# schmidtjonathan/Climate2Weather

Hardware: AMD Instinct MI355X
Metric: UNet denoise steps/sec (train fwd+bwd+allreduce+AdamW+EMA windows/s) (higher is better)
Workload: dtype bf16; 1 GPU; configs/sda_unet.yml default net, 5 vars x window 13 = 65 ch, 128x128, bf16 training step, 128 windows/GPU/step; global_batch=128, parallelism=dp1, params=72132929

## Files before the change

climate2weather_amd/_lib.py:

```python
from __future__ import annotations

import ctypes
import os
from ctypes import POINTER, Structure, c_char_p, c_float, c_int, c_int32, c_longlong, c_ulonglong, c_void_p

HERE = os.path.dirname(os.path.abspath(__file__))
LIB_PATH = os.environ.get("C2W_LIB") or os.path.join(HERE, "libc2w_hip.so")

DTYPE_F32, DTYPE_BF16, DTYPE_F16 = 0, 1, 2
CONV_1X1, CONV_S1, CONV_S2, CONV_UP, CONV_TS2 = 0, 1, 2, 3, 4
ACT_NONE, ACT_SILU, ACT_SILU_PAIR, ACT_RELU, ACT_RELU_PAIR = 0, 1, 2, 3, 4
MUL_PLAIN, MUL_DSILU = 0, 1
CONV_POOL2, CONV_WPACKED, CONV_NO_Y = 1, 2, 4
KERNEL_GATHER, KERNEL_PATCH_8X16, KERNEL_PATCH_16X16, KERNEL_PATCH_PAIR, KERNEL_PATCH_TS2, KERNEL_PATCH_S2 = 0, 1, 2, 3, 4, 5


class C2wError(RuntimeError):
    pass


class ConvArgs(Structure):
    _fields_ = [
        ("x", c_void_p), ("w", c_void_p), ("bias", c_void_p), ("res", c_void_p), ("mul", c_void_p), ("y", c_void_p), ("y2", c_void_p),
        ("B", c_int32), ("Hin", c_int32), ("Win", c_int32), ("Cin", c_int32),
        ("Hout", c_int32), ("Wout", c_int32), ("Cout", c_int32), ("ldy", c_int32),
        ("wrows", c_int32), ("mode", c_int32), ("act", c_int32), ("mulmode", c_int32),
        ("ln_x", c_void_p), ("ln_m", c_void_p), ("ln_dm", c_void_p), ("ln_ldm", c_int32), ("ln_unbiased", c_int32),
        ("ln_eps", c_float), ("flags", c_int32), ("lnf_y", c_void_p), ("lnf_m", c_void_p), ("kvalid", c_int32),
        ("lnf_rstd", c_void_p), ("ln_rstd", c_void_p),
        ("lnf_mean", c_void_p), ("res_rstd", c_void_p), ("res_mean", c_void_p), ("res_m", c_void_p),
        ("loss_sum", c_void_p), ("loss_scaler", c_void_p), ("loss_eps", c_void_p), ("loss_gscale", c_float), ("loss_C", c_int32),
        ("loss_lde", c_int32), ("splitk_ws", c_void_p), ("splitk_ws_bytes", c_ulonglong), ("splitk", c_int32),
    ]


class WgradItem(Structure):
    _fields_ = [("x", c_void_p), ("dy", c_void_p), ("dw", c_void_p), ("dbias", c_void_p)]


_PROTOS = {
    "c2w_conv_forward": [POINTER(ConvArgs), c_int, c_int, c_void_p],
    "c2w_conv_lnbwd_supported": [POINTER(ConvArgs), c_int],
    "c2w_conv_lnfwd_supported": [POINTER(ConvArgs), c_int],
    "c2w_conv_loss_supported": [POINTER(ConvArgs), c_int],
    "c2w_conv_splitk_plan": [POINTER(ConvArgs), c_int, POINTER(c_ulonglong)],
    "c2w_conv_lnfwd_chain_supported": [POINTER(ConvArgs), c_int],
    "c2w_conv_patch_supported": [POINTER(ConvArgs), c_int],
# ... 23 lines not shown
    "c2w_windows_to_nhwc_noise": [c_void_p, c_void_p, c_ulonglong, c_void_p, c_void_p, c_int, c_int, c_int, c_int, c_int, c_void_p],
    "c2w_mse_loss_grad_noise": [c_void_p, c_ulonglong, c_void_p, c_void_p, c_int, c_int, c_int, c_int, c_float, c_void_p, c_int, c_void_p],
    "c2w_sq_err": [c_void_p, c_void_p, c_void_p, c_void_p, c_int, c_int, c_int, c_int, c_int, c_void_p],
    "c2w_sq_err_noise": [c_void_p, c_ulonglong, c_void_p, c_void_p, c_int, c_int, c_int, c_int, c_int, c_void_p],
    "c2w_timestep_embedding": [c_void_p, c_void_p, c_int, c_int, c_float, c_void_p],
    "c2w_mu_sigma": [c_void_p, c_void_p, c_int, c_float, c_void_p],
    "c2w_publish_scalar": [c_void_p, c_void_p, c_int, c_void_p],
    "c2w_gemv_f32": [c_void_p, c_void_p, c_void_p, c_void_p, c_int, c_int, c_int, c_int, c_void_p],
    "c2w_conv_center_supported": [c_int, c_int, c_int, c_int, c_int],
    "c2w_conv_center": [c_void_p, c_void_p, c_void_p, c_void_p, c_int, c_int, c_int, c_int, c_int, c_int, c_int, c_longlong, c_int, c_void_p],
    "c2w_cast_f32": [c_void_p, c_void_p, c_longlong, c_int, c_void_p],
    "c2w_weight_transpose": [c_void_p, c_void_p, c_int, c_int, c_int, c_int, c_int, c_int, c_int, c_void_p],
    "c2w_weight_transpose_batched": [c_void_p, c_void_p, c_void_p, c_int, c_int, c_void_p],
    "c2w_pack_conv_weights_batched": [c_void_p, c_void_p, c_void_p, c_int, c_int, c_void_p],
    "c2w_conv_wpacked_supported": [POINTER(ConvArgs), c_int],
    "c2w_adamw_ema": [c_void_p, c_void_p, c_void_p, c_void_p, c_void_p, c_void_p, c_longlong, c_float, c_float, c_float, c_float,
                      c_float, c_int, c_float, c_float, c_void_p],
    "c2w_adamw_ema_scaled": [c_void_p, c_void_p, c_void_p, c_void_p, c_void_p, c_void_p, c_int, c_longlong, c_float, c_float, c_float,
                             c_float, c_float, c_int, c_float, c_float, c_void_p, c_void_p],
    "c2w_grad_scaler_init": [c_void_p, c_float, c_void_p],
    "c2w_grad_scaler_check": [c_void_p, c_longlong, c_void_p, c_void_p],
    "c2w_grad_scaler_update": [c_void_p, c_float, c_float, c_int, c_void_p],
    "c2w_ema_update": [c_void_p, c_void_p, c_longlong, c_float, c_void_p],
    "c2w_attention_forward": [c_void_p, c_void_p, c_void_p, c_int, c_int, c_int, c_int, c_void_p],
    "c2w_attention_backward": [c_void_p, c_void_p, c_void_p, c_void_p, c_void_p, c_void_p, c_int, c_int, c_int, c_int, c_void_p],
    "c2w_window_gather": [c_void_p, c_void_p, c_int, c_int, c_int, c_int, c_int, c_int, c_int, c_void_p],
    "c2w_window_scatter": [c_void_p, c_void_p, c_int, c_int, c_int, c_int, c_int, c_int, c_int, c_int, c_void_p],
    "c2w_sampler_predict": [c_void_p, c_void_p, c_void_p, c_longlong, c_float, c_float, c_void_p],
    "c2w_sumsq": [c_void_p, c_void_p, c_longlong, c_void_p],
    "c2w_sampler_correct": [c_void_p, c_void_p, c_void_p, c_void_p, c_void_p, c_longlong, c_float, c_float, c_void_p],
# ... 56 lines not shown
```

climate2weather_amd/csrc/conv_igemm.hip:

```cpp
#include <cstdlib>

#include "conv_epilogue.h"
#include "knobs.h"

namespace {

constexpr int BN = 128;
constexpr int WBYTES = BN * 128;
constexpr int NSLOT = 3;
template <int NW> struct GCfg {
    static constexpr int BM = 64 * NW;
    static constexpr int NTHREADS = 128 * NW;
    static constexpr int PBYTES = BM * 128;
    static constexpr int ROWS_PER_ROUND = NTHREADS / 8;
    static constexpr int WROUNDS = BN / ROWS_PER_ROUND;
    static constexpr int ROUND_BYTES = NTHREADS * 16;
};

template <typename T> struct Mma;
template <> struct Mma<bf16_t> {
    __device__ static __forceinline__ void run(const u32x4_t& a, const u32x4_t& b, f32x4_t& c) { c = mfma16<bf16_t>(a, b, c); }
};
template <> struct Mma<f16_t> {
    __device__ static __forceinline__ void run(const u32x4_t& a, const u32x4_t& b, f32x4_t& c) { c = mfma16<f16_t>(a, b, c); }
// ... 354 lines not shown
    return c2w_knobs().ln_chain && a->mode == C2W_CONV_S1 && c2w_conv_patch3_wanted(*a, dtype) ? 1 : 0;
}

extern "C" int c2w_conv_loss_supported(const C2wConvArgs* a, int dtype) {
    if (a == nullptr || (dtype != C2W_DTYPE_BF16 && dtype != C2W_DTYPE_F16)) return 0;
    if (a->mode != C2W_CONV_S1 || a->wrows > 80 || a->Cout > 128 || a->ldy != 128 || a->res != nullptr || a->mul != nullptr || a->y2 != nullptr ||
        a->act != C2W_ACT_NONE || a->ln_x != nullptr || a->lnf_y != nullptr || (a->flags & C2W_CONV_POOL2) != 0)
        return 0;
    if (a->loss_sum != nullptr && (a->loss_eps == nullptr || a->loss_C <= 0 || a->loss_C > a->wrows || (a->loss_lde & 7) != 0 || a->loss_lde < a->loss_C ||
                                   a->loss_lde > 128))
        return 0;
    const C2wKnobs& k = c2w_knobs();
    return !k.force_gather && k.loss_fusion && k.wgrad_narrow && c2w_conv_patch_eligible(*a) && c2w_conv_patch3_wanted(*a, dtype) ? 1 : 0;
}

extern "C" int c2w_conv_wpacked_supported(const C2wConvArgs* a, int dtype) {
    if (a == nullptr || (dtype != C2W_DTYPE_BF16 && dtype != C2W_DTYPE_F16)) return 0;
    return !c2w_knobs().force_gather && c2w_knobs().wpacked && c2w_conv_patch_eligible(*a) && c2w_conv_patch3_wanted(*a, dtype) ? 1 : 0;
}

extern "C" int c2w_conv_dispatch(const C2wConvArgs* a, int dtype) {
    if (a == nullptr) return C2W_ERR_BAD_ARG;
    const bool gather = c2w_knobs().force_gather;
    if (!gather && c2w_conv_patch_eligible(*a)) return c2w_conv_patch3_wanted(*a, dtype) ? C2W_KERNEL_PATCH_16X16 : C2W_KERNEL_PATCH_8X16;
    if (!gather && c2w_conv_pair_eligible(*a)) return C2W_KERNEL_PATCH_PAIR;
    if (!gather && c2w_conv_ts2_patch_eligible(*a)) return C2W_KERNEL_PATCH_TS2;
    if (!gather && c2w_conv_s2_patch_eligible(*a, dtype)) return C2W_KERNEL_PATCH_S2;
    return C2W_KERNEL_GATHER;
}

// ... 12 lines not shown
    if (a->lnf_y != nullptr && (naive != 0 || !c2w_conv_lnfwd_supported(a, dtype))) return C2W_ERR_BAD_SHAPE;
    if ((a->ln_rstd != nullptr && a->ln_x == nullptr) || (a->lnf_rstd != nullptr && a->lnf_y == nullptr)) return C2W_ERR_BAD_ARG;
    if (a->lnf_mean != nullptr || a->res_rstd != nullptr || a->res_mean != nullptr || a->res_m != nullptr || (a->flags & C2W_CONV_NO_Y) != 0) {
        if (a->lnf_y == nullptr || (a->res_rstd == nullptr) != (a->res_mean == nullptr) || (a->res_m != nullptr && a->res_rstd == nullptr) ||
            (a->res_rstd != nullptr && a->res == nullptr))
            return C2W_ERR_BAD_ARG;
        if (naive != 0 || !c2w_conv_lnfwd_chain_supported(a, dtype)) return C2W_ERR_BAD_SHAPE;
    }
    if ((a->flags & C2W_CONV_POOL2) != 0 && (naive != 0 || !c2w_conv_pool2_supported(a, dtype))) return C2W_ERR_BAD_SHAPE;
    if (a->loss_sum != nullptr && (naive != 0 || !c2w_conv_loss_supported(a, dtype))) return C2W_ERR_BAD_SHAPE;
    if (a->splitk > 1) {
        unsigned long long need = 0;
        if (naive != 0 || a->splitk_ws == nullptr || c2w_conv_splitk_plan_impl(*a, dtype, &need) != a->splitk || a->splitk_ws_bytes < need) return C2W_ERR_BAD_SHAPE;
    }
    if ((a->flags & C2W_CONV_WPACKED) != 0 && (naive != 0 || !c2w_conv_wpacked_supported(a, dtype))) return C2W_ERR_BAD_SHAPE;
    const bool patch = naive == 0 && !c2w_knobs().force_gather;
    if (patch && c2w_conv_patch_eligible(*a)) return c2w_conv_patch_s1(*a, dtype, st);
    if (patch && c2w_conv_pair_eligible(*a)) return c2w_conv_patch_pair(*a, dtype, st);
    if (patch && c2w_conv_ts2_patch_eligible(*a)) return c2w_conv_patch_ts2(*a, dtype, st);
    if (patch && c2w_conv_s2_patch_eligible(*a, dtype)) return c2w_conv_patch_s2(*a, dtype, st);
    if (naive == 2) naive = 0;
    if (dtype == C2W_DTYPE_F32) return launch_dtype<float>(*a, naive, st);
    if (dtype == C2W_DTYPE_BF16) return launch_dtype<bf16_t>(*a, naive, st);
    if (dtype == C2W_DTYPE_F16) return launch_dtype<f16_t>(*a, naive, st);
    return C2W_ERR_BAD_ARG;
}
```

climate2weather_amd/csrc/conv_patch3.hip:

```cpp
#include <cstdlib>

#include "conv_epilogue.h"
#include "knobs.h"

namespace {

constexpr int T3_WAVES = 8;
constexpr int T3_PW = 20;
constexpr int T3_WBYTES = 128 * 64;
constexpr int T3_OS = 128 * 2 + 16;

template <int TR, int NW = 4> struct T3Cfg {
    static constexpr int NTHR = 64 * NW;
    static constexpr int NPIECE = ((TR + 2) * T3_PW + 7) / 8;
    static constexpr int PBYTES = NPIECE * 1024;
    static constexpr int ROUNDS = (NPIECE + NW - 1) / NW;
    static constexpr int WPIECES = 8 / NW;
    static constexpr int NB = TR / (2 * NW);
    static constexpr int NPASS = TR / 8;
    static constexpr int LDS_LOOP = PBYTES + 3 * T3_WBYTES;
    static constexpr int LDS_EPI = TR * 16 * T3_OS + 512;
    static constexpr int LDS_BIAS = LDS_LOOP > LDS_EPI ? LDS_LOOP : LDS_EPI;
    static constexpr int LDS = LDS_BIAS + 1024;
    static constexpr int WAVES_PER_SIMD = NW == 8 ? 4 : (TR == 8 ? 3 : 2);
    static_assert(NB >= 1 && 8 % NW == 0, "wave tiling");
// ... 2 lines not shown
template <int N> struct IC3 { static constexpr int value = N; };


__device__ __forceinline__ uint32_t t3_pswz(int col) { return (uint32_t)(col & 7); }
__device__ __forceinline__ uint32_t t3_wswz(int row) { return (uint32_t)((4 - ((row >> 2) & 3)) & 3); }

template <int WPIECES> __device__ __forceinline__ void t3_wait(bool more) {
    if (more) {
        if constexpr (WPIECES == 2) asm volatile("s_waitcnt vmcnt(2)" ::: "memory");
        else asm volatile("s_waitcnt vmcnt(1)" ::: "memory");
    } else {
        asm volatile("s_waitcnt vmcnt(0)" ::: "memory");
    }
}

template <int TR, typename T = bf16_t, int NW = 4, int EPI = 0, bool WPK = false>
__global__ __launch_bounds__(64 * NW, (T3Cfg<TR, NW>::WAVES_PER_SIMD)) void conv_patch_t3_kernel(const C2wConvArgs p) {
    static_assert(sizeof(T) == 2, "16-bit storage types only");
    typedef T3Cfg<TR, NW> CF;
    constexpr int T3_NTHR = CF::NTHR;
    constexpr int ESZ = 2;
    constexpr int NB = CF::NB;
    extern __shared__ __attribute__((aligned(16))) char smem[];

    const int tid = threadIdx.x;
    const int lane = tid & 63;
    const int wid = __builtin_amdgcn_readfirstlane(tid >> 6);
    const int li = lane & 15, lg = lane >> 4;
    constexpr bool NARROW = EPI == 5 || EPI == 7;
    const int wm = NARROW ? wid >> 2 : wid & 1, wn = NARROW ? wid & 3 : wid >> 1;
    const bool light = NARROW && wid >= 4;
// ... 45 lines not shown
        if (NARROW && wid >= 5) return;
        if constexpr (wpk) {
            const uint32_t so = (uint32_t)(((tap * (p.Cin >> 5) + chunk * 2 + half) * (nN * 128) + co0) * 64);
#pragma unroll
            for (int i = 0; i < CF::WPIECES; ++i)
                glds16(rw, smem + CF::PBYTES + wslot * T3_WBYTES + (i * NW + wid) * 1024, (uint32_t)(i * NW * 1024 + tid * 16), so);
            return;
        }
        const uint32_t so = (uint32_t)(tap * p.Cin + chunk * 64 + half * 32) * ESZ;
#pragma unroll
        for (int i = 0; i < CF::WPIECES; ++i) glds16(rw, smem + CF::PBYTES + wslot * T3_WBYTES + (i * NW + wid) * 1024, wvo_at(i), so);
    };

    const uint32_t offA_held = (uint32_t)(CF::PBYTES + (wm * 64 + li) * 64 + (((uint32_t)lg ^ t3_wswz(li)) << 4));
    auto offA_at = [&]() {
        if constexpr (!(WPK && (EPI == 3 || EPI == 6))) return offA_held;
        int l = lane;
        asm volatile("" : "+v"(l));
        const int li_ = l & 15;
        return (uint32_t)(CF::PBYTES + (wm * 64 + li_) * 64 + (((uint32_t)(l >> 4) ^ t3_wswz(li_)) << 4));
    };
    auto offB_at = [&](int kw) {
        int l = lane;
        const int px = (l & 15) + kw;
        return (uint32_t)((wn * 4 * NB * T3_PW + px) * 128 + (((uint32_t)(l >> 4) ^ t3_pswz(px)) << 4));
    };

    f32x4_t acc[NB][4][4];
#pragma unroll
    for (int j = 0; j < NB; ++j)
#pragma unroll
        for (int m = 0; m < 4; ++m)
#pragma unroll
            for (int n = 0; n < 4; ++n) acc[j][m][n] = (f32x4_t){0.f, 0.f, 0.f, 0.f};
    const int kv = p.kvalid > 0 && p.kvalid < p.Cin ? p.kvalid : p.Cin;
    const int nhalf = (kv + 31) >> 5;
    const int NS = nhalf * 9;

    float bv[4][4];
    if (wid == 0) {
        const bool hb = p.bias != nullptr && co0 < p.wrows;
        const __amdgpu_buffer_rsrc_t rb = make_rsrc(hb ? (const void*)(p.bias + co0) : (const void*)p.w, hb ? (uint32_t)(p.wrows - co0) * 4u : 0u);
        glds16(rb, smem + CF::LDS_BIAS, lane < 32 ? (uint32_t)lane * 16u : C2W_OOB, 0u);
    }
    issue_patch(0);
    issue_w(0, 0, 0, 0);
    issue_w(0, 3, 0, 1);

    u32x4_t bq[4 * NB + 2];
    auto stage = [&](auto IDXc, int hc) {
        constexpr int IDX = decltype(IDXc)::value;
        constexpr int KW = IDX / 3;
        constexpr int KH = IDX % 3;
        constexpr int WS = IDX % 3;
        const int s = hc * 9 + IDX;
        const int half = hc & 1, c = hc >> 1;
        auto issue_ahead = [&]() {
            constexpr int I2 = (IDX + 2) % 9;
            constexpr int T2 = (I2 % 3) * 3 + I2 / 3;
            const int h2 = IDX + 2 < 9 ? hc : hc + 1;
            issue_w(h2 >> 1, T2, h2 & 1, I2 % 3);
        };
// ... 135 lines not shown
        if (!pool2) est.prefetch_tile16(p, tid_e, co0, ((long long)b * H + oh0 + 8 * h) * W + ow0, W);
        __syncthreads();
        const char* const Oh = O + h * 128 * T3_OS;
        if constexpr (EPI == 2 || EPI == 8) est.template finish_lnf<EPI == 8>(p, Oh, T3_OS, tid_e, b);
        else if constexpr (EPI == 3 || EPI == 6) est.finish_ln(p, Oh, T3_OS, tid_e, b, red);
        else if constexpr (EPI == 4) est.finish(p, Oh, T3_OS, tid_e);
        else if (pool2) est.finish_pool2(p, Oh, T3_OS, tid_e, co0, ((long long)b * (H >> 1) + ((oh0 + 8 * h) >> 1)) * (W >> 1) + (ow0 >> 1), W >> 1);
        else if (p.ln_x != nullptr) est.finish_ln(p, Oh, T3_OS, tid_e, b, red);
        else if (p.lnf_y != nullptr) est.finish_lnf(p, Oh, T3_OS, tid_e, b);
        else est.finish(p, Oh, T3_OS, tid_e);
        if (h + 1 < CF::NPASS) __syncthreads();
    }
    }
}

template <int TR, typename T, int NW, int EPI, bool WPK>
int t3_launch_wpk(const C2wConvArgs& a, hipStream_t st) {
    typedef T3Cfg<TR, NW> CF;
    static bool attr = false;
    if (!attr) {
        HIP_CHECK_RET(hipFuncSetAttribute((const void*)conv_patch_t3_kernel<TR, T, NW, EPI, WPK>, hipFuncAttributeMaxDynamicSharedMemorySize, CF::LDS));
        attr = true;
    }
    const int nN = (a.Cout + 127) / 128;
    const int nM = a.B * (a.Hout / TR) * (a.Wout >> 4);
    conv_patch_t3_kernel<TR, T, NW, EPI, WPK><<<nM * nN, CF::NTHR, CF::LDS, st>>>(a);
    return (int)hipGetLastError();
}
template <int TR, typename T, int NW, int EPI>
int t3_launch_as(const C2wConvArgs& a, hipStream_t st) {
    return (a.flags & C2W_CONV_WPACKED) != 0 ? t3_launch_wpk<TR, T, NW, EPI, true>(a, st) : t3_launch_wpk<TR, T, NW, EPI, false>(a, st);
}

template <int TR, typename T, int NW>
int t3_launch(const C2wConvArgs& a, hipStream_t st) {
    if (TR == 16 && (a.flags & C2W_CONV_POOL2) == 0) {
        if (a.lnf_y != nullptr) return a.res_rstd != nullptr ? t3_launch_as<16, T, NW, 8>(a, st) : t3_launch_as<16, T, NW, 2>(a, st);
        if (a.ln_x != nullptr) return a.ln_rstd != nullptr ? t3_launch_as<16, T, NW, 6>(a, st) : t3_launch_as<16, T, NW, 3>(a, st);
        if (a.loss_sum != nullptr) return t3_launch_as<16, T, NW, 7>(a, st);
        if (a.wrows <= 80 && a.Cout <= 128 && c2w_knobs().wgrad_narrow) return t3_launch_as<16, T, NW, 5>(a, st);
        return t3_launch_as<16, T, NW, 4>(a, st);
    }
    return t3_launch_as<TR, T, NW, 0>(a, st);
}

}

bool c2w_conv_patch3_wanted(const C2wConvArgs& a, int dtype) {
    const int mode = c2w_knobs().conv_t3;
    if ((dtype != C2W_DTYPE_BF16 && dtype != C2W_DTYPE_F16) || mode == 0 || (a.Hout & 15) != 0 || (a.Wout & 15) != 0) return false;
// ... 8 lines not shown
```

climate2weather_amd/engine.py:

```python
from __future__ import annotations

import os

from dataclasses import dataclass
from typing import Callable, Dict, List, Optional, Tuple

import torch

from . import ops
from .nn import BlockSpec, LevelSpec
from .ops import (ACT_NONE, ACT_RELU, ACT_RELU_PAIR, ACT_SILU, ACT_SILU_PAIR, CONV_1X1, CONV_S1, CONV_S2, CONV_TS2, CONV_UP, DTYPE_BF16, DTYPE_F16, DTYPE_F32, MUL_DSILU, MUL_PLAIN, TORCH_DTYPE)

import weakref

LN_EPS = 1e-5
_ENGINE_BY_PARAM_ID: Dict[int, "weakref.ReferenceType"] = {}


def engine_of_parameter(p):
    ref = _ENGINE_BY_PARAM_ID.get(id(p))
    eng = ref() if ref is not None else None
    if eng is None:
        _ENGINE_BY_PARAM_ID.pop(id(p), None)
        return None
# ... 161 lines not shown
        self._pk_ok: Dict[tuple, bool] = {}
        self._pk_want: Dict[tuple, dict] = {}
        self._pk_desc: Dict[tuple, torch.Tensor] = {}
        self._pk_sync: Dict[tuple, list] = {}
        self.use_packed_weights = os.environ.get("C2W_NO_WPACKED") is None
        self._gwpad: Dict[str, torch.Tensor] = {}
        self._manual_ver = 0
        self._wg_stream = None
        self.prefetch_dgrad = os.environ.get("C2W_NO_DG_PREFETCH") is None and \
            (os.environ.get("C2W_WGRAD_STREAM", "0") == "1" or os.environ.get("C2W_DG_PREFETCH") == "1")
        self._dg_ready = None
        self.use_grad_stream = os.environ.get("C2W_WGRAD_STREAM", "0") == "1"
        self._wgrad_behind = max(0, int(os.environ.get("C2W_WGRAD_BEHIND", "0") or 0))
        self._wg_pending = []
        self.keep_ln_stats = os.environ.get("C2W_NO_LN_STATS") != "1"
        _grp = os.environ.get("C2W_WGRAD_GROUP", "64")
        self.group_wgrads = _grp != "0"
        self.group_wgrads_max_side = int(_grp) if _grp.isdigit() and int(_grp) > 1 else 1 << 30
        self.group_wgrads_top = max(1, int(os.environ.get("C2W_WGRAD_GROUP_TOP", "1")))
        self._wg_groups: Dict[tuple, list] = {}
        self._wg_group_ok: Dict[tuple, bool] = {}
        self._done_releases: list = []
        self._pub = None
        self._skip_dw = False
        self._ws: Dict[int, torch.Tensor] = {}
        self._splitk_plans: Dict[tuple, tuple] = {}
        self.debug_trace: Optional[list] = None
        self.attach(net)

    def attach(self, net) -> None:
# ... 15 lines not shown
        for i in self._bound_by_id:
            _ENGINE_BY_PARAM_ID[i] = me
        self.generation = getattr(self, "generation", 0) + 1
        self._slots, self._slots_net, self._links = None, (lambda: None), []
        self._offs4 = [4 * off for off, _, _ in lay.views.values()]
        self._pver = self._param_versions()
        self.flat = flat
        self.flat_grad = None
        self.shadows.clear()
        self.dg.clear()
        self.dg_lin = None
        self._shadow_ver.clear()
        self._dg_ver.clear()
        self._dg_desc.clear()
        self._wpad.clear()
        self._pk.clear()
        self._pk_tab.clear()
        self._pk_ok.clear()
        self._pk_want.clear()
        self._pk_desc.clear()
        self._pk_sync.clear()
        self._gwpad.clear()

    def is_attached(self, net) -> bool:
        if self.flat is None:
            return False
        slots = self._slots
        if slots is None or self._slots_net() is not net:
            slots = self._slots = [_resolve(net, name) for name in self.layout.views]
            self._slots_net = weakref.ref(net)
# ... 174 lines not shown
        self._dg_ready = ev

    def _conv_weights(self, kind: str, rec: ConvRec, dt: int, g: dict, fused_ln_bwd: bool = False):
        plain = self._w(rec, dt) if kind == "f" else self._wT(rec, dt)
        if not self.use_packed_weights or dt == DTYPE_F32:
            return plain, False
        key = (kind, rec.name, dt, g["B"], g["Hin"], g["Win"], g["Hout"], g["Wout"], g["Cout"], g["mode"], ops.KNOBS_GENERATION)
        ok = self._pk_ok.get(key)
        if ok is None:
            ok = self._pk_ok[key] = bool(ops.conv_wpacked_supported(g, dt))
        if not ok:
            return plain, False
        pk = self._packed(kind, rec, dt)
        return (pk, True) if pk is not None else (plain, False)

    def _gw(self, rec: ConvRec) -> torch.Tensor:
        return self.flat_grad[rec.w_off:]

    def _gb(self, rec: ConvRec) -> torch.Tensor:
        return self.flat_grad[rec.b_off:]

    def grad_stream(self):
        if self.flat is None or not self.flat.is_cuda or not self.use_grad_stream:
            return None
        return self.side_stream()

    def side_stream(self):
        if self.flat is None or not self.flat.is_cuda:
            return None
        if self._wg_stream is None or self._wg_stream.device != self.flat.device:
# ... 250 lines not shown
                done = regen and x.data.is_contiguous() and x.data.dtype == torch.float32 and \
                    ops.windows_to_nhwc_noise(x.data, x.offsets(), noise[0], noise[1], x0, B, C, H * W, lay.cin_pad, dt)
                if not done:
                    x = x.materialize().contiguous().float()
            if done:
                pass
            elif regen:
                if not ops.nchw_to_nhwc_noise(x, noise[0], noise[1], x0, B, C, H * W, lay.cin_pad, dt):
                    eps = torch.empty_like(x)
                    ops.philox_normal(eps, eps.numel(), noise[0])
                    ops.nchw_to_nhwc(x, eps, noise[1], x0, B, C, H * W, lay.cin_pad, dt)
            else:
                ops.nchw_to_nhwc(x, noise[0] if noise else None, noise[1] if noise else None, x0, B, C, H * W, lay.cin_pad, dt)

        def conv3(name, xin, Hi, Wi, Ho, Wo, mode, act=ACT_NONE, res=None, ldy=None, cout=None, y2=None, want_ln=None, loss=None,
                  resn=None, no_y=False):
            rec = lay.convs[name]
            ldy_ = ldy or rec.rows
            y = torch.empty((B * Ho * Wo, ldy_), dtype=T, device=dev) if not no_y else None
            g = self._geom(B, Hi, Wi, rec.kstride, Ho, Wo, cout or rec.rows, ldy_, rec.rows, mode)
            hn = None
            lnf = None
            if want_ln is not None and act == ACT_NONE and y2 is None and ops.conv_lnfwd_supported(g, dt):
                hn = torch.empty((B * Ho * Wo, ldy_), dtype=T, device=dev)
                lnf = dict(y=hn, m=want_ln[1], ldm=ldm if want_ln[1] is not None else 0, eps=LN_EPS, unbiased=self.ln_unbiased)
                if train and self.keep_ln_stats and want_ln[0] == "mod":
                    lnf["rstd"] = hn._c2w_rstd = torch.empty((B * Ho * Wo,), dtype=torch.float32, device=dev)
                if no_y:
                    lnf["mean"] = hn._c2w_mean = torch.empty((B * Ho * Wo,), dtype=torch.float32, device=dev)
            if no_y or resn is not None:
                assert lnf is not None and (not no_y or "rstd" in lnf), "chain form without a fused LayerNorm (run_blocks decides both from the same answers)"
            wop, wpk = self._conv_weights("f", rec, dt, g)
            ops.conv(xin, wop, self._b(rec), y if y is not None else hn, g, dt, act=act, res=res, y2=y2, lnf=lnf,
                     kvalid=rec.cin if rec.kstride != rec.cin else 0, wpacked=wpk, loss=loss, resn=resn, no_y=no_y,
                     splitk=self._splitk(g, dt, act) if (not train and lnf is None and y2 is None and loss is None and not wpk) else None)
            if self.debug_trace is not None and y is not None:
                self.debug_trace.append((name, y, dict(x=xin, w=self._w(rec, dt), g=g, act=act, res=res)))
                if hn is not None:
                    self.debug_trace.append((name + " [LayerNorm emitted]", hn))
            if want_ln is not None:
                return y, g, rec, hn
            return y, g, rec

        def dgrad(rec, gy, Hi, Wi, Ho, Wo, mode, ld_out, mul=None, res=None, ln=None, mulmode=MUL_DSILU):
            g = self._geom(B, Hi, Wi, rec.dg_ld, Ho, Wo, ld_out, ld_out, rec.cin, mode)
            if ln is not None and not ops.conv_lnbwd_supported(g, dt):
                return None
            dx = torch.empty((B * Ho * Wo, ld_out), dtype=T, device=dev)
            wop, wpk = self._conv_weights("d", rec, dt, g, fused_ln_bwd=ln is not None)
            ops.conv(gy, wop, None, dx, g, dt, res=res, mul=mul, mulmode=mulmode, ln=ln,
                     kvalid=rec.rows if rec.dg_ld != rec.rows else 0, wpacked=wpk)
            return dx

        def res_block(b: BlockSpec, xin, Hc, Wc, h0=None, want_ln=None, elide=False):
            p = "unet." + b.key
            Cc = b.channels
            npix = B * Hc * Wc
            m = m_all.view(-1)[b.mod_offset:]
            rstd0 = getattr(h0, "_c2w_rstd", None) if h0 is not None else None
            if xin is None:
                assert rstd0 is not None and getattr(h0, "_c2w_mean", None) is not None
            if h0 is None:
                h0 = torch.empty((npix, Cc), dtype=T, device=dev)
                ops.ln_forward(xin, m, h0, npix, Hc * Wc, Cc, ldm, LN_EPS, self.ln_unbiased, dt)
            d1 = torch.empty((npix, Cc), dtype=T, device=dev) if train else None
            mulmode = MUL_PLAIN
# ... 58 lines not shown
                    ops.conv(dqkv, self._wT(rq, dt), None, dhl, self._geom(npix, 1, 1, 3 * Cc, 1, 1, Cc, Cc, Cc, CONV_1X1), dt)
                    tape.done(rq.w_off)
                    dx = torch.empty_like(dhl)
                    ops.ln_backward(dhl, xin, None, gy, dx, None, npix, Tn, Cc, 0, LN_EPS, self.ln_unbiased, dt)
                    return dx
                tape.steps.append(bw)
            return out

        Hc, Wc = H, W
        lv0 = lay.levels[0]
        def mod_of(b: BlockSpec):
            return ("mod", m_all.view(-1)[b.mod_offset:])

        first0 = lv0.descent[0] if lv0.descent else None
        if first0 is not None and first0.kind == "res":
            cur, g_h0, r_h0, hn0 = conv3("unet." + lv0.head_key, x0, H, W, H, W, CONV_S1, want_ln=mod_of(first0))
        else:
            (cur, g_h0, r_h0), hn0 = conv3("unet." + lv0.head_key, x0, H, W, H, W, CONV_S1), None
        if train:
            def bw_head0(gy, x0=x0, g=g_h0, rec=r_h0):
                self.flush_wgrad_groups()
                self._wgrad(rec, x0, gy, g, dt)
                dx0 = dgrad(rec, gy, H, W, H, W, CONV_S1, lay.cin_pad) if want_dx else None
                tape.done(rec.w_off)
                return dx0
            tape.steps.append(bw_head0)
        def chain_ok(Cc, Hc, Wc):
            g = self._geom(B, Hc, Wc, Cc, Hc, Wc, Cc, Cc, Cc, CONV_S1)
            return dt != DTYPE_F32 and ops.conv_lnfwd_chain_supported(g, dt) and ops.conv_lnbwd_supported(g, dt)

        def run_blocks(blocks, cur, Hc, Wc, h0, tail_ln):
            hn = h0

# ... 72 lines not shown
            else:
                xin = cur
                if fold is not None and not train and nhwc_out and self._fold_output(fold, "unet." + lv.tail_key, xin, B, Hc, Wc, dt):
                    return None
                lfuse = None
                if loss_rows is not None:
                    lfuse = dict(sum=loss["sum"], gscale=loss["gscale"], scaler=loss.get("scaler"), eps=loss_rows[0], lde=loss_rows[1], C=lay.out_channels)
                cur, g_t, r_t = conv3("unet." + lv.tail_key, xin, Hc, Wc, Hc, Wc, CONV_S1, ldy=lay.cout_pad, cout=lay.cout_pad, loss=lfuse)
                if train:
                    tape.meta["loss_fused"] = lfuse is not None
                if train:
                    def bw_tail0(gy, xin=xin, g=g_t, rec=r_t, Hc=Hc, Wc=Wc, Cc=lv.channels):
                        gw = dict(g)
                        gw["Cout"] = rec.rows
                        self._wg(xin, gy, rec, gw, dt)
                        dxt = dgrad(rec, gy, Hc, Wc, Hc, Wc, CONV_S1, Cc)
                        tape.done(rec.w_off)
                        return dxt
                    tape.steps.append(bw_tail0)
        if train:
            tape.meta.update(B=B, C=C, H=H, W=W, dt=dt, out_nhwc=cur, ldm=ldm, Bt=Bt)
        if nhwc_out:
            return cur
        y = torch.empty((B, C, H, W), dtype=torch.float32, device=dev)
        ops.nhwc_to_nchw(cur, y, B, lay.out_channels, H * W, lay.cout_pad, dt)
        return y

    use_center_conv = os.environ.get("C2W_NO_CENTER_CONV") != "1"
    chain_blocks = os.environ.get("C2W_LN_CHAIN") == "1"
    use_splitk = os.environ.get("C2W_NO_SPLITK") is None
    fuse_loss = os.environ.get("C2W_NO_LOSS_FUSION") is None
# ... 167 lines not shown
```

climate2weather_amd/ops.py:

```python
from __future__ import annotations

import ctypes
from typing import Optional

import torch

from . import _lib
from ._lib import (ACT_NONE, ACT_RELU, ACT_RELU_PAIR, ACT_SILU, ACT_SILU_PAIR, CONV_1X1, CONV_S1, CONV_S2, CONV_TS2, CONV_UP, DTYPE_BF16, DTYPE_F16, DTYPE_F32, MUL_DSILU,
                   MUL_PLAIN, ConvArgs, check)

TORCH_DTYPE = {DTYPE_F32: torch.float32, DTYPE_BF16: torch.bfloat16, DTYPE_F16: torch.float16}
ESZ = {DTYPE_F32: 4, DTYPE_BF16: 2, DTYPE_F16: 2}
CK = {DTYPE_F32: 32, DTYPE_BF16: 64, DTYPE_F16: 64}


def _p(t: Optional[torch.Tensor]):
    if t is None:
        return None
    if not t.is_cuda:
        raise _lib.C2wError("climate2weather_amd kernels need GPU tensors (no CPU fallback in the product path)")
    return ctypes.c_void_p(t.data_ptr())


def _stream():
# ... 7 lines not shown
        a.ln_x, a.ln_m, a.ln_dm = _p(ln["x"]), _p(ln.get("m")), _p(ln.get("dm"))
        a.ln_ldm, a.ln_unbiased, a.ln_eps = int(ln.get("ldm", 0)), int(ln["unbiased"]), float(ln["eps"])
        a.ln_rstd = _p(ln.get("rstd"))
    if lnf is not None:
        a.lnf_y, a.lnf_m = _p(lnf["y"]), _p(lnf.get("m"))
        a.lnf_rstd = _p(lnf.get("rstd"))
        a.lnf_mean = _p(lnf.get("mean"))
        a.ln_ldm, a.ln_unbiased, a.ln_eps = int(lnf.get("ldm", 0)), int(lnf["unbiased"]), float(lnf["eps"])
    if resn is not None:
        a.res_rstd, a.res_mean, a.res_m = _p(resn["rstd"]), _p(resn["mean"]), _p(resn.get("m"))
    return a


def conv(x, w, bias, y, g: dict, dtype: int, act: int = ACT_NONE, res=None, mul=None, mulmode: int = MUL_PLAIN, naive=False, y2=None,
         ln=None, lnf=None, pool2: bool = False, kvalid: int = 0, wpacked: bool = False, loss: Optional[dict] = None,
         resn: Optional[dict] = None, no_y: bool = False, splitk: Optional[tuple] = None):
    a = _conv_args(x, w, bias, res, mul, y, g, act, mulmode, y2, ln, lnf, resn)
    if no_y:
        a.flags |= _lib.CONV_NO_Y
    if pool2:
        a.flags |= _lib.CONV_POOL2
    if wpacked:
        a.flags |= _lib.CONV_WPACKED
    a.kvalid = int(kvalid)
    if splitk is not None:
        ws, ns = splitk
        a.splitk_ws, a.splitk_ws_bytes, a.splitk = _p(ws), ws.numel() * ws.element_size(), int(ns)
    if loss is not None:
        a.loss_sum, a.loss_scaler = _p(loss["sum"]), _p(loss.get("scaler"))
        a.loss_eps, a.loss_lde, a.loss_gscale, a.loss_C = _p(loss["eps"]), int(loss["lde"]), float(loss["gscale"]), int(loss["C"])
    check(_lib.load().c2w_conv_forward(ctypes.byref(a), dtype, int(naive), _stream()), "c2w_conv_forward")


def conv_wpacked_supported(g: dict, dtype: int) -> bool:
    a = ConvArgs(None, None, None, None, None, None, None, g["B"], g["Hin"], g["Win"], g["Cin"], g["Hout"], g["Wout"], g["Cout"], g["ldy"],
                 g["wrows"], g["mode"], ACT_NONE, MUL_PLAIN)
    return bool(_lib.load().c2w_conv_wpacked_supported(ctypes.byref(a), dtype))


def packed_conv_weights_numel(rows: int, cin: int) -> int:
    return 9 * cin * ((rows + 127) // 128 * 128)


def pack_conv_weights_batched(src, dst, desc, n: int, dtype: int) -> None:
    check(_lib.load().c2w_pack_conv_weights_batched(_p(src), _p(dst), _p(desc), n, dtype, _stream()), "c2w_pack_conv_weights_batched")

# ... 343 lines not shown
```

include/c2w_hip.h:

```cpp
#ifndef C2W_HIP_H
#define C2W_HIP_H
#include <stddef.h>
#include <stdint.h>

#ifdef __cplusplus
extern "C" {
#endif

enum { C2W_DTYPE_F32 = 0, C2W_DTYPE_BF16 = 1, C2W_DTYPE_F16 = 2 };
enum { C2W_ERR_BAD_ARG = -1, C2W_ERR_BAD_SHAPE = -2, C2W_ERR_UNSUPPORTED = -3 };

enum {
    C2W_CONV_1X1 = 0,
    C2W_CONV_S1 = 1,
    C2W_CONV_S2 = 2,
    C2W_CONV_UP = 3,
    C2W_CONV_TS2 = 4
};
enum { C2W_ACT_NONE = 0, C2W_ACT_SILU = 1, C2W_ACT_SILU_PAIR = 2, C2W_ACT_RELU = 3, C2W_ACT_RELU_PAIR = 4 };
enum { C2W_MUL_PLAIN = 0, C2W_MUL_DSILU = 1 };
enum { C2W_CONV_POOL2 = 1, C2W_CONV_WPACKED = 2, C2W_CONV_NO_Y = 4 };

typedef struct C2wConvArgs {
    const void* x;
// ... 22 lines not shown
    float* lnf_rstd;
    const float* ln_rstd;
    float* lnf_mean;
    const float* res_rstd;
    const float* res_mean;
    const float* res_m;
    float* loss_sum;
    const float* loss_scaler;
    const void* loss_eps;
    float loss_gscale;
    int32_t loss_C;
    int32_t loss_lde;
    float* splitk_ws;
    unsigned long long splitk_ws_bytes;
    int32_t splitk;
} C2wConvArgs;

int c2w_conv_patch_supported(const C2wConvArgs* args, int dtype);
int c2w_conv_pool2_supported(const C2wConvArgs* args, int dtype);
int c2w_conv_lnfwd_supported(const C2wConvArgs* args, int dtype);
int c2w_conv_lnbwd_supported(const C2wConvArgs* args, int dtype);
int c2w_conv_lnfwd_chain_supported(const C2wConvArgs* args, int dtype);
int c2w_conv_loss_supported(const C2wConvArgs* args, int dtype);
int c2w_conv_splitk_plan(const C2wConvArgs* args, int dtype, unsigned long long* ws_bytes);

enum { C2W_KERNEL_GATHER = 0, C2W_KERNEL_PATCH_8X16 = 1, C2W_KERNEL_PATCH_16X16 = 2, C2W_KERNEL_PATCH_PAIR = 3, C2W_KERNEL_PATCH_TS2 = 4, C2W_KERNEL_PATCH_S2 = 5 };
int c2w_conv_dispatch(const C2wConvArgs* args, int dtype);
int c2w_conv_wgrad_dispatch(const C2wConvArgs* args, int dtype);

int c2w_conv_forward(const C2wConvArgs* args, int dtype, int naive, void* stream);

int c2w_conv_wgrad(const C2wConvArgs* args, float* dw, float* dbias, void* workspace, unsigned long long workspace_bytes, int dtype,
                   void* stream);
long long c2w_conv_wgrad_workspace_bytes(const C2wConvArgs* args, int dtype);
// ... 98 lines not shown
```

Before: 2742 windows/s.

## Handle odd trailing input channel of head conv with a separate tap stage

For 3x3 stride-1 convs whose real input channel count is a multiple of 64 plus one (the 65-channel head conv and its dgrad tail), the kernel now runs its K loop only over the 64-aligned channels. The single leftover channel is handled by a small extra stage that loads an 18x18 halo of that channel plus a packed 9-tap weight slice into LDS and folds it into the accumulators with extra MFMAs. The goal is to avoid processing a nearly empty 32-channel K chunk padded from one channel. The cost is extra LDS, a cached permuted tap-weight buffer rebuilt whenever the weights change, and a new launch variant with hand-counted vmcnt waits.

```diff
diff --git a/climate2weather_amd/_lib.py b/climate2weather_amd/_lib.py
--- a/climate2weather_amd/_lib.py
+++ b/climate2weather_amd/_lib.py
@@ -31,6 +31,7 @@
         ("lnf_mean", c_void_p), ("res_rstd", c_void_p), ("res_mean", c_void_p), ("res_m", c_void_p),
         ("loss_sum", c_void_p), ("loss_scaler", c_void_p), ("loss_eps", c_void_p), ("loss_gscale", c_float), ("loss_C", c_int32),
         ("loss_lde", c_int32), ("splitk_ws", c_void_p), ("splitk_ws_bytes", c_ulonglong), ("splitk", c_int32),
+        ("taps_w", c_void_p), ("taps_c", c_int32),
     ]
 
 
@@ -84,6 +85,7 @@
     "c2w_weight_transpose_batched": [c_void_p, c_void_p, c_void_p, c_int, c_int, c_void_p],
     "c2w_pack_conv_weights_batched": [c_void_p, c_void_p, c_void_p, c_int, c_int, c_void_p],
     "c2w_conv_wpacked_supported": [POINTER(ConvArgs), c_int],
+    "c2w_conv_taps_supported": [POINTER(ConvArgs), c_int],
     "c2w_adamw_ema": [c_void_p, c_void_p, c_void_p, c_void_p, c_void_p, c_void_p, c_longlong, c_float, c_float, c_float, c_float,
                       c_float, c_int, c_float, c_float, c_void_p],
     "c2w_adamw_ema_scaled": [c_void_p, c_void_p, c_void_p, c_void_p, c_void_p, c_void_p, c_int, c_longlong, c_float, c_float, c_float,
diff --git a/climate2weather_amd/csrc/conv_igemm.hip b/climate2weather_amd/csrc/conv_igemm.hip
--- a/climate2weather_amd/csrc/conv_igemm.hip
+++ b/climate2weather_amd/csrc/conv_igemm.hip
@@ -392,6 +392,19 @@
     return !k.force_gather && k.loss_fusion && k.wgrad_narrow && c2w_conv_patch_eligible(*a) && c2w_conv_patch3_wanted(*a, dtype) ? 1 : 0;
 }
 
+extern "C" int c2w_conv_taps_supported(const C2wConvArgs* a, int dtype) {
+    if (a == nullptr || (dtype != C2W_DTYPE_BF16 && dtype != C2W_DTYPE_F16)) return 0;
+    if (a->mode != C2W_CONV_S1 || a->Hin != a->Hout || a->Win != a->Wout) return 0;
+    if (a->taps_c <= 0 || (a->taps_c & 63) != 0 || a->taps_c >= a->Cin || a->kvalid != a->taps_c + 1) return 0;
+    if (a->ln_x != nullptr || a->loss_sum != nullptr || a->res_rstd != nullptr || a->lnf_mean != nullptr || (a->flags & (C2W_CONV_POOL2 | C2W_CONV_NO_Y)) != 0 ||
+        a->splitk > 1)
+        return 0;
+    const C2wKnobs& k = c2w_knobs();
+    if (a->lnf_y == nullptr && a->wrows <= 80 && a->Cout <= 128 && k.wgrad_narrow) return 0;
+    if (a->lnf_y != nullptr && !c2w_conv_lnfwd_supported(a, dtype)) return 0;
+    return !k.force_gather && c2w_conv_patch_eligible(*a) && c2w_conv_patch3_wanted(*a, dtype) ? 1 : 0;
+}
+
 extern "C" int c2w_conv_wpacked_supported(const C2wConvArgs* a, int dtype) {
     if (a == nullptr || (dtype != C2W_DTYPE_BF16 && dtype != C2W_DTYPE_F16)) return 0;
     return !c2w_knobs().force_gather && c2w_knobs().wpacked && c2w_conv_patch_eligible(*a) && c2w_conv_patch3_wanted(*a, dtype) ? 1 : 0;
@@ -434,6 +447,7 @@
         if (naive != 0 || a->splitk_ws == nullptr || c2w_conv_splitk_plan_impl(*a, dtype, &need) != a->splitk || a->splitk_ws_bytes < need) return C2W_ERR_BAD_SHAPE;
     }
     if ((a->flags & C2W_CONV_WPACKED) != 0 && (naive != 0 || !c2w_conv_wpacked_supported(a, dtype))) return C2W_ERR_BAD_SHAPE;
+    if (a->taps_w != nullptr && (naive != 0 || !c2w_conv_taps_supported(a, dtype))) return C2W_ERR_BAD_SHAPE;
     const bool patch = naive == 0 && !c2w_knobs().force_gather;
     if (patch && c2w_conv_patch_eligible(*a)) return c2w_conv_patch_s1(*a, dtype, st);
     if (patch && c2w_conv_pair_eligible(*a)) return c2w_conv_patch_pair(*a, dtype, st);
diff --git a/climate2weather_amd/csrc/conv_patch3.hip b/climate2weather_amd/csrc/conv_patch3.hip
--- a/climate2weather_amd/csrc/conv_patch3.hip
+++ b/climate2weather_amd/csrc/conv_patch3.hip
@@ -9,6 +9,7 @@
 constexpr int T3_PW = 20;
 constexpr int T3_WBYTES = 128 * 64;
 constexpr int T3_OS = 128 * 2 + 16;
+constexpr int T3_TBYTES = 512 * 16;
 
 template <int TR, int NW = 4> struct T3Cfg {
     static constexpr int NTHR = 64 * NW;
@@ -41,7 +42,7 @@
     }
 }
 
-template <int TR, typename T = bf16_t, int NW = 4, int EPI = 0, bool WPK = false>
+template <int TR, typename T = bf16_t, int NW = 4, int EPI = 0, bool WPK = false, bool TAPS = false>
 __global__ __launch_bounds__(64 * NW, (T3Cfg<TR, NW>::WAVES_PER_SIMD)) void conv_patch_t3_kernel(const C2wConvArgs p) {
     static_assert(sizeof(T) == 2, "16-bit storage types only");
     typedef T3Cfg<TR, NW> CF;
@@ -117,7 +118,7 @@
 
     const uint32_t offA_held = (uint32_t)(CF::PBYTES + (wm * 64 + li) * 64 + (((uint32_t)lg ^ t3_wswz(li)) << 4));
     auto offA_at = [&]() {
-        if constexpr (!(WPK && (EPI == 3 || EPI == 6))) return offA_held;
+        if constexpr (!((WPK && (EPI == 3 || EPI == 6)) || TAPS)) return offA_held;
         int l = lane;
         asm volatile("" : "+v"(l));
         const int li_ = l & 15;
@@ -137,7 +138,7 @@
 #pragma unroll
             for (int n = 0; n < 4; ++n) acc[j][m][n] = (f32x4_t){0.f, 0.f, 0.f, 0.f};
     const int kv = p.kvalid > 0 && p.kvalid < p.Cin ? p.kvalid : p.Cin;
-    const int nhalf = (kv + 31) >> 5;
+    const int nhalf = TAPS ? p.taps_c >> 5 : (kv + 31) >> 5;
     const int NS = nhalf * 9;
 
     float bv[4][4];
@@ -146,9 +147,46 @@
         const __amdgpu_buffer_rsrc_t rb = make_rsrc(hb ? (const void*)(p.bias + co0) : (const void*)p.w, hb ? (uint32_t)(p.wrows - co0) * 4u : 0u);
         glds16(rb, smem + CF::LDS_BIAS, lane < 32 ? (uint32_t)lane * 16u : C2W_OOB, 0u);
     }
+    if constexpr (TAPS) {
+        const int f = wid * 64 + lane, hr = f / 18, hc_ = f - hr * 18;
+        const int ih = oh0 - 1 + hr, iw = ow0 - 1 + hc_;
+        const bool ok = f < 18 * 18 && (unsigned)ih < (unsigned)H && (unsigned)iw < (unsigned)W;
+        glds16(rx, smem + CF::LDS + wid * 1024, ok ? (uint32_t)((ih * Ws + iw) * p.Cin + p.taps_c) * ESZ : C2W_OOB, 0u);
+        const __amdgpu_buffer_rsrc_t rtw = make_rsrc(p.taps_w, (uint32_t)p.wrows * 64u);
+#pragma unroll
+        for (int i = 0; i < CF::WPIECES; ++i)
+            glds16(rtw, smem + CF::PBYTES + 2 * T3_WBYTES + (i * NW + wid) * 1024, (uint32_t)(i * NW * 1024 + tid * 16), (uint32_t)co0 * 64u);
+    }
     issue_patch(0);
     issue_w(0, 0, 0, 0);
     issue_w(0, 3, 0, 1);
+    if constexpr (TAPS) {
+        static_assert(!NARROW || !TAPS, "tap stage: wide epilogue families only");
+        static_assert(CF::ROUNDS + 2 * CF::WPIECES == 8, "vmcnt below");
+        asm volatile("s_waitcnt vmcnt(8)" ::: "memory");
+        __builtin_amdgcn_s_barrier();
+        u32x4_t a[4];
+        const uint32_t offA = offA_at() + 2u * T3_WBYTES;
+#pragma unroll
+        for (int m = 0; m < 4; ++m) a[m] = *(const u32x4_t*)(smem + offA + m * 1024);
+        int tl = tid;
+        asm volatile("" : "+v"(tl));
+        const int li_t = tl & 15;
+        const bool odd = ((tl >> 4) & 1) != 0;
+#pragma unroll
+        for (int n = 0; n < 4 * NB; ++n) {
+            const int r = wn * 4 * NB + n;
+            uint32_t h[8];
+#pragma unroll
+            for (int e = 0; e < 8; ++e) {
+                const int slot = odd ? (e == 0 ? (r + 2) * 18 + li_t + 2 : 511) : (r + e / 3) * 18 + li_t + e % 3;
+                h[e] = *(const uint16_t*)(smem + CF::LDS + slot * 16);
+            }
+            const u32x4_t bt = {h[0] | (h[1] << 16), h[2] | (h[3] << 16), h[4] | (h[5] << 16), h[6] | (h[7] << 16)};
+#pragma unroll
+            for (int m = 0; m < 4; ++m) acc[n >> 2][m][n & 3] = mfma16<T>(a[m], bt, acc[n >> 2][m][n & 3]);
+        }
+    }
 
     u32x4_t bq[4 * NB + 2];
     auto stage = [&](auto IDXc, int hc) {
@@ -314,26 +352,33 @@
     }
 }
 
-template <int TR, typename T, int NW, int EPI, bool WPK>
+template <int TR, typename T, int NW, int EPI, bool WPK, bool TAPS = false>
 int t3_launch_wpk(const C2wConvArgs& a, hipStream_t st) {
     typedef T3Cfg<TR, NW> CF;
+    constexpr int LDS = CF::LDS + (TAPS ? T3_TBYTES : 0);
+    static_assert(2 * LDS <= 160 * 1024, "two workgroups per CU");
     static bool attr = false;
     if (!attr) {
-        HIP_CHECK_RET(hipFuncSetAttribute((const void*)conv_patch_t3_kernel<TR, T, NW, EPI, WPK>, hipFuncAttributeMaxDynamicSharedMemorySize, CF::LDS));
+        HIP_CHECK_RET(hipFuncSetAttribute((const void*)conv_patch_t3_kernel<TR, T, NW, EPI, WPK, TAPS>, hipFuncAttributeMaxDynamicSharedMemorySize, LDS));
         attr = true;
     }
     const int nN = (a.Cout + 127) / 128;
     const int nM = a.B * (a.Hout / TR) * (a.Wout >> 4);
-    conv_patch_t3_kernel<TR, T, NW, EPI, WPK><<<nM * nN, CF::NTHR, CF::LDS, st>>>(a);
+    conv_patch_t3_kernel<TR, T, NW, EPI, WPK, TAPS><<<nM * nN, CF::NTHR, LDS, st>>>(a);
     return (int)hipGetLastError();
 }
 template <int TR, typename T, int NW, int EPI>
 int t3_launch_as(const C2wConvArgs& a, hipStream_t st) {
     return (a.flags & C2W_CONV_WPACKED) != 0 ? t3_launch_wpk<TR, T, NW, EPI, true>(a, st) : t3_launch_wpk<TR, T, NW, EPI, false>(a, st);
 }
+template <int TR, typename T, int NW, int EPI>
+int t3_launch_taps(const C2wConvArgs& a, hipStream_t st) {
+    return (a.flags & C2W_CONV_WPACKED) != 0 ? t3_launch_wpk<TR, T, NW, EPI, true, true>(a, st) : t3_launch_wpk<TR, T, NW, EPI, false, true>(a, st);
+}
 
 template <int TR, typename T, int NW>
 int t3_launch(const C2wConvArgs& a, hipStream_t st) {
+    if (TR == 16 && a.taps_w != nullptr) return a.lnf_y != nullptr ? t3_launch_taps<16, T, NW, 2>(a, st) : t3_launch_taps<16, T, NW, 4>(a, st);
     if (TR == 16 && (a.flags & C2W_CONV_POOL2) == 0) {
         if (a.lnf_y != nullptr) return a.res_rstd != nullptr ? t3_launch_as<16, T, NW, 8>(a, st) : t3_launch_as<16, T, NW, 2>(a, st);
         if (a.ln_x != nullptr) return a.ln_rstd != nullptr ? t3_launch_as<16, T, NW, 6>(a, st) : t3_launch_as<16, T, NW, 3>(a, st);
diff --git a/climate2weather_amd/engine.py b/climate2weather_amd/engine.py
--- a/climate2weather_amd/engine.py
+++ b/climate2weather_amd/engine.py
@@ -199,6 +199,9 @@
         self._wgrad_behind = max(0, int(os.environ.get("C2W_WGRAD_BEHIND", "0") or 0))
         self._wg_pending = []
         self.keep_ln_stats = os.environ.get("C2W_NO_LN_STATS") != "1"
+        self.edge_taps = os.environ.get("C2W_EDGE_TAPS", "1") != "0"
+        self._taps_ok: Dict[tuple, bool] = {}
+        self._tapw: Dict[tuple, tuple] = {}
         _grp = os.environ.get("C2W_WGRAD_GROUP", "64")
         self.group_wgrads = _grp != "0"
         self.group_wgrads_max_side = int(_grp) if _grp.isdigit() and int(_grp) > 1 else 1 << 30
@@ -244,6 +247,7 @@
         self._dg_ver.clear()
         self._dg_desc.clear()
         self._wpad.clear()
+        self._tapw.clear()
         self._pk.clear()
         self._pk_tab.clear()
         self._pk_ok.clear()
@@ -448,6 +452,29 @@
         pk = self._packed(kind, rec, dt)
         return (pk, True) if pk is not None else (plain, False)
 
+    def _edge_taps(self, kind: str, rec: ConvRec, g: dict, dt: int, lnf: bool = False) -> Optional[dict]:
+        ld, c = (rec.kstride, rec.cin - 1) if kind == "f" else (rec.dg_ld, rec.rows - 1)
+        if not self.edge_taps or ops.EMULATED or dt == DTYPE_F32 or ld == c + 1 or c <= 0 or c % 64 != 0:
+            return None
+        key = (kind, rec.name, dt, g["B"], g["Hin"], g["Win"], g["Hout"], g["Wout"], g["Cout"], g["mode"], lnf, ops.KNOBS_GENERATION)
+        ok = self._taps_ok.get(key)
+        if ok is None:
+            ok = self._taps_ok[key] = bool(ops.conv_taps_supported(g, dt, c, lnf=lnf))
+        return dict(w=self._tap_weights(kind, rec, dt), c=c) if ok else None
+
+    def _tap_weights(self, kind: str, rec: ConvRec, dt: int) -> torch.Tensor:
+        key = (kind, rec.name, dt)
+        ent = self._tapw.get(key)
+        if ent is None or ent[0] != self._version():
+            if kind == "f":
+                rows, w9 = rec.rows, self._w(rec, dt)[: rec.rows * rec.taps * rec.kstride].view(rec.rows, rec.taps, rec.kstride)[:, :, rec.cin - 1]
+            else:
+                rows, w9 = rec.cin, self._wT(rec, dt)[: rec.cin * rec.taps * rec.dg_ld].view(rec.cin, rec.taps, rec.dg_ld)[:, :, rec.rows - 1]
+            buf = ent[1] if ent is not None else torch.empty((_round_up(rows, 128), 32), dtype=TORCH_DTYPE[dt], device=self.flat.device)
+            ops.tap_weights(w9, buf)
+            self._tapw[key] = ent = (self._version(), buf)
+        return ent[1]
+
     def _gw(self, rec: ConvRec) -> torch.Tensor:
         return self.flat_grad[rec.w_off:]
 
@@ -728,7 +755,7 @@
                 ops.nchw_to_nhwc(x, noise[0] if noise else None, noise[1] if noise else None, x0, B, C, H * W, lay.cin_pad, dt)
 
         def conv3(name, xin, Hi, Wi, Ho, Wo, mode, act=ACT_NONE, res=None, ldy=None, cout=None, y2=None, want_ln=None, loss=None,
-                  resn=None, no_y=False):
+                  resn=None, no_y=False, edge=False):
             rec = lay.convs[name]
             ldy_ = ldy or rec.rows
             y = torch.empty((B * Ho * Wo, ldy_), dtype=T, device=dev) if not no_y else None
@@ -745,9 +772,11 @@
             if no_y or resn is not None:
                 assert lnf is not None and (not no_y or "rstd" in lnf), "chain form without a fused LayerNorm (run_blocks decides both from the same answers)"
             wop, wpk = self._conv_weights("f", rec, dt, g)
+            taps = self._edge_taps("f", rec, g, dt, lnf=lnf is not None) if edge and train and rec.kstride != rec.cin else None
             ops.conv(xin, wop, self._b(rec), y if y is not None else hn, g, dt, act=act, res=res, y2=y2, lnf=lnf,
                      kvalid=rec.cin if rec.kstride != rec.cin else 0, wpacked=wpk, loss=loss, resn=resn, no_y=no_y,
-                     splitk=self._splitk(g, dt, act) if (not train and lnf is None and y2 is None and loss is None and not wpk) else None)
+                     splitk=self._splitk(g, dt, act) if (not train and lnf is None and y2 is None and loss is None and not wpk) else None,
+                     **({"taps": taps} if taps is not None else {}))
             if self.debug_trace is not None and y is not None:
                 self.debug_trace.append((name, y, dict(x=xin, w=self._w(rec, dt), g=g, act=act, res=res)))
                 if hn is not None:
@@ -756,14 +785,15 @@
                 return y, g, rec, hn
             return y, g, rec
 
-        def dgrad(rec, gy, Hi, Wi, Ho, Wo, mode, ld_out, mul=None, res=None, ln=None, mulmode=MUL_DSILU):
+        def dgrad(rec, gy, Hi, Wi, Ho, Wo, mode, ld_out, mul=None, res=None, ln=None, mulmode=MUL_DSILU, edge=False):
             g = self._geom(B, Hi, Wi, rec.dg_ld, Ho, Wo, ld_out, ld_out, rec.cin, mode)
             if ln is not None and not ops.conv_lnbwd_supported(g, dt):
                 return None
             dx = torch.empty((B * Ho * Wo, ld_out), dtype=T, device=dev)
             wop, wpk = self._conv_weights("d", rec, dt, g, fused_ln_bwd=ln is not None)
+            taps = self._edge_taps("d", rec, g, dt) if edge and ln is None and rec.dg_ld != rec.rows else None
             ops.conv(gy, wop, None, dx, g, dt, res=res, mul=mul, mulmode=mulmode, ln=ln,
-                     kvalid=rec.rows if rec.dg_ld != rec.rows else 0, wpacked=wpk)
+                     kvalid=rec.rows if rec.dg_ld != rec.rows else 0, wpacked=wpk, **({"taps": taps} if taps is not None else {}))
             return dx
 
         def res_block(b: BlockSpec, xin, Hc, Wc, h0=None, want_ln=None, elide=False):
@@ -852,9 +882,9 @@
 
         first0 = lv0.descent[0] if lv0.descent else None
         if first0 is not None and first0.kind == "res":
-            cur, g_h0, r_h0, hn0 = conv3("unet." + lv0.head_key, x0, H, W, H, W, CONV_S1, want_ln=mod_of(first0))
+            cur, g_h0, r_h0, hn0 = conv3("unet." + lv0.head_key, x0, H, W, H, W, CONV_S1, want_ln=mod_of(first0), edge=True)
         else:
-            (cur, g_h0, r_h0), hn0 = conv3("unet." + lv0.head_key, x0, H, W, H, W, CONV_S1), None
+            (cur, g_h0, r_h0), hn0 = conv3("unet." + lv0.head_key, x0, H, W, H, W, CONV_S1, edge=True), None
         if train:
             def bw_head0(gy, x0=x0, g=g_h0, rec=r_h0):
                 self.flush_wgrad_groups()
@@ -957,7 +987,7 @@
                         gw = dict(g)
                         gw["Cout"] = rec.rows
                         self._wg(xin, gy, rec, gw, dt)
-                        dxt = dgrad(rec, gy, Hc, Wc, Hc, Wc, CONV_S1, Cc)
+                        dxt = dgrad(rec, gy, Hc, Wc, Hc, Wc, CONV_S1, Cc, edge=True)
                         tape.done(rec.w_off)
                         return dxt
                     tape.steps.append(bw_tail0)
diff --git a/climate2weather_amd/ops.py b/climate2weather_amd/ops.py
--- a/climate2weather_amd/ops.py
+++ b/climate2weather_amd/ops.py
@@ -45,7 +45,7 @@
 
 def conv(x, w, bias, y, g: dict, dtype: int, act: int = ACT_NONE, res=None, mul=None, mulmode: int = MUL_PLAIN, naive=False, y2=None,
          ln=None, lnf=None, pool2: bool = False, kvalid: int = 0, wpacked: bool = False, loss: Optional[dict] = None,
-         resn: Optional[dict] = None, no_y: bool = False, splitk: Optional[tuple] = None):
+         resn: Optional[dict] = None, no_y: bool = False, splitk: Optional[tuple] = None, taps: Optional[dict] = None):
     a = _conv_args(x, w, bias, res, mul, y, g, act, mulmode, y2, ln, lnf, resn)
     if no_y:
         a.flags |= _lib.CONV_NO_Y
@@ -60,7 +60,31 @@
     if loss is not None:
         a.loss_sum, a.loss_scaler = _p(loss["sum"]), _p(loss.get("scaler"))
         a.loss_eps, a.loss_lde, a.loss_gscale, a.loss_C = _p(loss["eps"]), int(loss["lde"]), float(loss["gscale"]), int(loss["C"])
+    if taps is not None:
+        a.taps_w, a.taps_c = _p(taps["w"]), int(taps["c"])
     check(_lib.load().c2w_conv_forward(ctypes.byref(a), dtype, int(naive), _stream()), "c2w_conv_forward")
+
+
+def conv_taps_supported(g: dict, dtype: int, taps_c: int, lnf: bool = False) -> bool:
+    a = _geom_args(g)
+    a.kvalid, a.taps_c = int(taps_c) + 1, int(taps_c)
+    a.lnf_y = 1 if lnf else None
+    return bool(_lib.load().c2w_conv_taps_supported(ctypes.byref(a), dtype))
+
+
+_TAP_PERM = {}
+
+
+def tap_weights(w9: torch.Tensor, out: torch.Tensor) -> None:
+    rows = out.shape[0]
+    key = (rows, out.device)
+    if key not in _TAP_PERM:
+        r = torch.arange(rows, device=out.device).view(rows, 1)
+        j = torch.arange(4, device=out.device).view(1, 4)
+        _TAP_PERM[key] = ((j ^ ((4 - ((r >> 2) & 3)) & 3)).view(rows, 4, 1) * 8 + torch.arange(8, device=out.device).view(1, 1, 8)).view(rows, 32)
+    logical = torch.zeros((rows, 32), dtype=out.dtype, device=out.device)
+    logical[: w9.shape[0], :9] = w9
+    out.copy_(torch.gather(logical, 1, _TAP_PERM[key]))
 
 
 def conv_wpacked_supported(g: dict, dtype: int) -> bool:
diff --git a/include/c2w_hip.h b/include/c2w_hip.h
--- a/include/c2w_hip.h
+++ b/include/c2w_hip.h
@@ -60,10 +60,13 @@
     float* splitk_ws;
     unsigned long long splitk_ws_bytes;
     int32_t splitk;
+    const void* taps_w;
+    int32_t taps_c;
 } C2wConvArgs;
 
 int c2w_conv_patch_supported(const C2wConvArgs* args, int dtype);
 int c2w_conv_pool2_supported(const C2wConvArgs* args, int dtype);
+int c2w_conv_taps_supported(const C2wConvArgs* args, int dtype);
 int c2w_conv_lnfwd_supported(const C2wConvArgs* args, int dtype);
 int c2w_conv_lnbwd_supported(const C2wConvArgs* args, int dtype);
 int c2w_conv_lnfwd_chain_supported(const C2wConvArgs* args, int dtype);
```

Result: no change. 2746 windows/s, median of 6 (+0.2%).
